# tensorlayer/TLXCV

Measured on AMD Instinct MI355X. Metric: images/sec fwd, higher is better.
Workload: dtype f16; 1 GPU; ResNet-50 fp16 forward, 224x224, batch 256 per GPU (BASELINE configs[1]); global_batch=256, per_gpu_batch=256, weights=seeded random (tlxcv_amd.seeded, seed 1), parallelism=single GPU, launch=hipGraph replay of the forward

## Files before the change

include/tlxmi.h:

```cpp
#ifndef TLXMI_H
#define TLXMI_H

#include <stddef.h>
#include <stdint.h>

#ifdef __cplusplus
extern "C" {
#endif

#define TLXMI_VERSION 101

typedef enum tlxmi_status {
    TLXMI_OK = 0,
    TLXMI_ERR_BAD_ARG = -1,
    TLXMI_ERR_UNSUPPORTED = -2,
    TLXMI_ERR_ALIGNMENT = -3,
    TLXMI_ERR_LAUNCH = -4,
    TLXMI_ERR_NO_DEVICE = -5
} tlxmi_status;

typedef enum tlxmi_dtype { TLXMI_F16 = 0, TLXMI_F32 = 1 } tlxmi_dtype;

typedef enum tlxmi_act {
    TLXMI_ACT_NONE = 0,
// ... 44 lines not shown
    int32_t R, S;
    int32_t stride_h, stride_w, pad_h, pad_w, dil_h, dil_w;
    int32_t Ho, Wo;
    int32_t x_ld, y_ld, res_ld;
    int32_t y_nstride;
    int32_t res_nstride;
    int32_t act;
    float act_param;
    uint32_t flags;
} tlxmi_conv2d_desc;

int tlxmi_conv2d(const tlxmi_conv2d_desc* d, const void* x, const void* w_packed,
                 const float* scale , const float* shift ,
                 const void* res , void* y, void* stream);
int tlxmi_conv2d_maxpool_supported(const tlxmi_conv2d_desc* d);

int tlxmi_yolo_iou_aware(const void* x, void* y, int dtype, int64_t pixels, int A, int C, float factor, void* stream);
int tlxmi_yolo_box(const void* x, int dtype, int N, int A, int C, int H, int W, int channels_last, const int32_t* img_size,
                   const float* anchors, float conf_thresh, int downsample_ratio, int clip_bbox, float scale_x_y,
                   float* boxes, float* scores, int Mtot, int m_offset, void* stream);
size_t tlxmi_multiclass_nms_workspace_bytes(int N, int M);
int tlxmi_multiclass_nms(const float* boxes, const float* scores, int N, int M, int C, float score_threshold, float nms_threshold,
                         int keep_top_k, void* workspace, float* detections, int32_t* counts, void* stream);
int tlxmi_multiclass_nms_index(const float* boxes, const float* scores, int N, int M, int C, float score_threshold,
                               float nms_threshold, int keep_top_k, void* workspace, float* detections, int32_t* counts,
                               int32_t* keep_index, void* stream);

typedef struct tlxmi_preproc_desc {
    int32_t N, H, W, C;
    int32_t out_h, out_w;
    int32_t kh, kw;
    int32_t out_dtype;
    int32_t layout;
    int32_t fold_b, cpad;
    int32_t normalize;
} tlxmi_preproc_desc;
size_t tlxmi_preprocess_u8_workspace_bytes(const tlxmi_preproc_desc* d);
int tlxmi_preprocess_u8(const tlxmi_preproc_desc* d, const void* images, const int32_t* xbounds, const int32_t* xk,
                        const int32_t* ybounds, const int32_t* yk, const float* mean, const float* std_, void* workspace,
                        void* out, void* stream);

int tlxmi_preprocess_linear_u8(const tlxmi_preproc_desc* d, const void* images, const int32_t* xidx, const int32_t* xcoef,
                               const int32_t* yidx, const int32_t* ycoef, const float* mean, const float* std_, void* out,
                               void* stream);

typedef struct tlxmi_seam_desc {
    int32_t dtype;
    int64_t rows;
    int32_t K1, N1, N2;
    int32_t t2_ld, skip_ld, y_ld, t1_ld;
    int32_t act;
} tlxmi_seam_desc;
int tlxmi_bottleneck_seam_supported(int dtype, int K1, int N1, int N2);
int tlxmi_bottleneck_seam_proj(const tlxmi_seam_desc* d, const void* t2, const void* w3_packed, const float* scale3,
                               const float* shift3, const void* x, const void* wd_packed, const float* scale_d,
                               const float* shift_d, void* y, const void* w1_packed, const float* scale1,
                               const float* shift1, void* t1, void* stream);
int tlxmi_bottleneck_seam(const tlxmi_seam_desc* d, const void* t2, const void* w3_packed, const float* scale3,
                          const float* shift3, const void* skip, void* y, const void* w1_packed, const float* scale1,
                          const float* shift1, void* t1, void* stream);
int tlxmi_bottleneck_seam_dec_supported(int dtype, int K1, int N1, int N2, int64_t rows, int H, int W);
int tlxmi_bottleneck_seam_dec(const tlxmi_seam_desc* d, int H, int W, const void* t2, const void* w3_packed, const float* scale3,
                              const float* shift3, const void* skip, void* y, const void* w1_packed, const float* scale1,
                              const float* shift1, void* t1, void* stream);

typedef struct tlxmi_proj_desc {
    int32_t dtype;
    int32_t N, Ho, Wo;
    int32_t K1, K2, Cout;
    int32_t H2, W2, stride;
    int32_t x_ld, x2_ld, y_ld;
    int32_t act;
    float act_param;
    uint32_t flags;
} tlxmi_proj_desc;
int tlxmi_conv1x1_proj_supported(const tlxmi_proj_desc* d, const void* x, const void* x2, const void* w_packed, const void* y);
int tlxmi_conv1x1_proj(const tlxmi_proj_desc* d, const void* x, const void* x2, const void* w_packed, const float* shift, void* y,
                       void* stream);

int tlxmi_group_conv_chunks(int Cin, int Cout, int groups, int dtype);
size_t tlxmi_packed_group_filter_bytes(int Cout, int Cin, int R, int S, int groups, int dtype);
int tlxmi_pack_group_filter(const float* src_oihw, void* dst, int Cout, int Cin, int R, int S, int groups,
                            int dtype, void* stream);
int tlxmi_group_conv2d(const tlxmi_conv2d_desc* d, int groups, const void* x, const void* w_packed,
                       const float* scale, const float* shift, const void* res, void* y, void* stream);
int tlxmi_group_conv2d_small_supported(const tlxmi_conv2d_desc* d, int groups);

int tlxmi_linear_splitk(int dtype, int64_t rows, int K, int Cout, int x_ld, const void* x, const void* w_packed,
                        int splits, void* partials, const float* scale, const float* shift, const void* res,
                        int res_ld, int act, float act_param, uint32_t flags, void* y, int y_ld, void* stream);

int tlxmi_conv2d_splitk_supported(const tlxmi_conv2d_desc* d, int splits);
int tlxmi_conv2d_splitk(const tlxmi_conv2d_desc* d, int splits, const void* x, const void* w_packed, void* partials,
                        const float* scale, const float* shift, const void* res, void* y, void* stream);

typedef struct tlxmi_dwconv2d_desc {
    int32_t dtype;
    int32_t N, H, W, C;
    int32_t R, S, stride_h, stride_w, pad_h, pad_w, dil_h, dil_w;
    int32_t Ho, Wo;
    int32_t x_ld, y_ld;
    int32_t act;
    float act_param;
} tlxmi_dwconv2d_desc;
int tlxmi_dwconv2d(const tlxmi_dwconv2d_desc* d, const void* x, const void* w_rsc, const float* scale,
                   const float* shift, void* y, void* stream);
// ... 222 lines not shown
```

tlxcv_amd/_lib.py:

```python
import ctypes as C
import os

_HERE = os.path.dirname(os.path.abspath(__file__))
LIB_PATH = os.path.join(_HERE, "libtlxmi.so")

F16, F32 = 0, 1
ACT_NONE, ACT_RELU, ACT_RELU6, ACT_LEAKY, ACT_HARDSWISH, ACT_HARDSIGMOID, ACT_GELU, ACT_SIGMOID, ACT_SILU = range(9)
EPI_RES_AFTER_ACT = 1
EPI_MAXPOOL_3S2P1 = 4
PLAN_SHARED_HALF = 0x100
PLAN_SHARED_FULL = 0x200
LAYOUT_NHWC, LAYOUT_NCHW = 0, 1


class ConvDesc(C.Structure):
    _fields_ = [(n, C.c_int32) for n in (
        "dtype", "N", "H", "W", "C", "Cout", "R", "S", "stride_h", "stride_w", "pad_h", "pad_w",
        "dil_h", "dil_w", "Ho", "Wo", "x_ld", "y_ld", "res_ld", "y_nstride", "res_nstride", "act")] + [
        ("act_param", C.c_float), ("flags", C.c_uint32)]


class DwConvDesc(C.Structure):
    _fields_ = [(n, C.c_int32) for n in (
        "dtype", "N", "H", "W", "C", "R", "S", "stride_h", "stride_w", "pad_h", "pad_w", "dil_h",
# ... 114 lines not shown
    "tlxmi_affine_act": [_vp, _vp, _vp, _vp, _vp, _i, _l, _i, _i, _i, _i, _i, _f, _u, _vp],
    "tlxmi_scale_channels": [_vp, _vp, _vp, _i, _i, _i, _i, _i, _i, _i, _vp],
    "tlxmi_layernorm": [_vp, _vp, _vp, _vp, _i, _l, _i, _i, _i, _f, _vp],
    "tlxmi_layernorm_window_partition": [_vp, _vp, _vp, _vp, _i, _i, _i, _i, _i, _i, _i, _f, _vp],
    "tlxmi_window_reverse_layernorm": [_vp, _vp, _vp, _vp, _vp, _vp, _i, _i, _i, _i, _i, _i, _i, _f, _vp],
    "tlxmi_mlp_seam": [_i, _l, _i, _i, _i, _vp, _i, _vp, _vp, _vp, _vp, _vp, _i, _vp, _i, _vp],
    "tlxmi_linear_stats": [_i, _l, _i, _i, _i, _i, _vp, _vp, _vp, _vp, _i, _vp, _vp, _u, _vp],
    "tlxmi_softmax_rows": [_vp, _vp, _i, _l, _i, _l, _l, _vp],
    "tlxmi_linear_ln": [_i, _l, _i, _i, _i, _i, _vp, _vp, _vp, _vp, _vp, _f, _i, _vp, _u, _vp],
    "tlxmi_attention": [C.POINTER(AttnDesc), _vp, _vp, _vp, _vp, _vp],
    "tlxmi_attention_comb": [C.POINTER(AttnDesc), _vp, _vp, _vp, _vp],
    "tlxmi_attention_windows": [C.POINTER(AttnDesc), _vp, _vp, _vp, _i, _i, _i, _i, _vp],
    "tlxmi_mha": [C.POINTER(MhaDesc), _vp, _vp, _vp, _vp, _vp, _vp, _vp],
    "tlxmi_sr_attention": [C.POINTER(MhaDesc), _vp, _vp, _vp, _vp, _vp],
    "tlxmi_cswin_attention": [C.POINTER(CswinAttnDesc), _vp, _vp, _vp, _vp, _vp, _vp, _vp],
    "tlxmi_cswin_attention_plain": [C.POINTER(CswinAttnDesc), _vp, _vp, _vp, _vp, _vp, _vp, _vp],
    "tlxmi_levit_attention": [C.POINTER(LevitAttnDesc), _vp, _vp, _vp, _vp, _vp, _vp],
    "tlxmi_levit_attention_plain": [C.POINTER(LevitAttnDesc), _vp, _vp, _vp, _vp, _vp, _vp],
    "tlxmi_tnt_inner": [C.POINTER(TntInnerDesc), _vp, _vp, _vp, _vp, _vp],
    "tlxmi_tnt_inner_plain": [C.POINTER(TntInnerDesc), _vp, _vp, _vp, _vp, _vp],
    "tlxmi_gsa_block": [C.POINTER(GsaBlockDesc), _vp, _vp, _vp, _vp, _vp, _vp],
    "tlxmi_window_partition": [_vp, _vp, _i, _i, _i, _i, _i, _i, _i, _vp],
    "tlxmi_window_reverse": [_vp, _vp, _vp, _i, _i, _i, _i, _i, _i, _i, _vp],
    "tlxmi_patch_merge_gather": [_vp, _vp, _i, _i, _i, _i, _i, _vp],
    "tlxmi_patch_merge_layernorm": [_vp, _vp, _vp, _vp, _i, _i, _i, _i, _i, _f, _vp],
    "tlxmi_upsample2x_nearest": [_vp, _vp, _i, _i, _i, _i, _i, _i, _i, _i, _vp],
    "tlxmi_copy_channels": [_vp, _vp, _i, _l, _i, _i, _i, _vp],
    "tlxmi_argmax_lastdim": [_vp, _i, _l, _i, _i, _vp, _vp],
    "tlxmi_resize_bilinear": [_vp, _i, _i, _i, _i, _i, _i, _vp, _i, _i, _i, _i, _i, _l, _i, C.c_double, C.c_double, _vp],
    "tlxmi_sepconv2d": [C.POINTER(SepConvDesc), _vp, _vp, _vp, _vp, _vp, _vp, _vp, _vp, _vp],
    "tlxmi_dwconv7_stats": [C.POINTER(DwConv7Desc), _vp, _vp, _vp, _vp, _vp, _vp],
    "tlxmi_preact_conv1x1": [_i, _l, _i, _i, _i, _i, _vp, _vp, _vp, _i, _vp, _vp, _vp, _i, _vp, _vp],
    "tlxmi_lka_dw": [C.POINTER(LkaDwDesc), _vp, _vp, _vp, _vp, _vp, _vp, _vp],
    "tlxmi_lka_gate": [C.POINTER(LkaGateDesc), _vp, _vp, _vp, _vp, _vp, _vp, _vp, _vp, _vp, _vp, _vp, _vp],
    "tlxmi_mul": [_vp, _vp, _vp, _i, _l, _i, _i, _i, _i, _vp],
    "tlxmi_shuffle_unit": [C.POINTER(ShuffleUnitDesc), _vp, _vp, _vp, _vp],
    "tlxmi_shuffle_concat": [_vp, _vp, _vp, _i, _l, _i, _i, _i, _i, _vp],
    "tlxmi_ghost_module": [C.POINTER(GhostModuleDesc), _vp, _vp, _vp, _vp, _vp],
}
_SPECIAL = {
    "tlxmi_version": ([], C.c_int),
    "tlxmi_last_error": ([], C.c_char_p),
    "tlxmi_device_count": ([], C.c_int),
    "tlxmi_packed_filter_bytes": ([_i, _i, _i, _i, _i], C.c_size_t),
    "tlxmi_packed_group_filter_bytes": ([_i, _i, _i, _i, _i, _i], C.c_size_t),
    "tlxmi_group_conv_chunks": ([_i, _i, _i, _i], C.c_int),
    "tlxmi_group_conv2d_small_supported": ([C.POINTER(ConvDesc), _i], C.c_int),
    "tlxmi_conv2d_maxpool_supported": ([C.POINTER(ConvDesc)], C.c_int),
    "tlxmi_conv2d_splitk_supported": ([C.POINTER(ConvDesc), _i], C.c_int),
    "tlxmi_preprocess_u8_workspace_bytes": ([C.POINTER(PreprocDesc)], C.c_size_t),
    "tlxmi_multiclass_nms_workspace_bytes": ([_i, _i], C.c_size_t),
    "tlxmi_bottleneck_seam_supported": ([_i, _i, _i, _i], C.c_int),
    "tlxmi_bottleneck_seam_dec_supported": ([_i, _i, _i, _i, _l, _i, _i], C.c_int),
    "tlxmi_conv1x1_proj_supported": ([C.POINTER(ProjDesc), _vp, _vp, _vp, _vp], C.c_int),
    "tlxmi_linear_ln_supported": ([_i, _l, _i, _i, _i, _i], C.c_int),
    "tlxmi_mlp_seam_supported": ([_i, _i, _i, _i], C.c_int),
    "tlxmi_sepconv2d_supported": ([C.POINTER(SepConvDesc)], C.c_int),
    "tlxmi_dwconv7_stats_supported": ([C.POINTER(DwConv7Desc)], C.c_int),
    "tlxmi_preact_conv1x1_supported": ([_i, _l, _i, _i, _i, _i, _i, _i], C.c_int),
    "tlxmi_sr_attention_supported": ([C.POINTER(MhaDesc)], C.c_int),
    "tlxmi_cswin_attention_supported": ([C.POINTER(CswinAttnDesc)], C.c_int),
    "tlxmi_levit_attention_supported": ([C.POINTER(LevitAttnDesc)], C.c_int),
    "tlxmi_tnt_inner_supported": ([C.POINTER(TntInnerDesc)], C.c_int),
    "tlxmi_tnt_inner_param_count": ([_i, _i], C.c_size_t),
    "tlxmi_gsa_block_supported": ([C.POINTER(GsaBlockDesc)], C.c_int),
    "tlxmi_gsa_block_param_count": ([_i], C.c_size_t),
    "tlxmi_lka_dw_supported": ([C.POINTER(LkaDwDesc)], C.c_int),
    "tlxmi_lka_gate_supported": ([C.POINTER(LkaGateDesc)], C.c_int),
    "tlxmi_shuffle_unit_supported": ([C.POINTER(ShuffleUnitDesc)], C.c_int),
    "tlxmi_shuffle_unit_param_bytes": ([_i], C.c_size_t),
    "tlxmi_ghost_module_supported": ([C.POINTER(GhostModuleDesc)], C.c_int),
    "tlxmi_ghost_module_param_bytes": ([_i, _i], C.c_size_t),
}
ALL_SYMBOLS = sorted(list(PROTOTYPES) + list(_SPECIAL))

TUNE_LIB_PATH = os.environ.get("TLXMI_TUNE_LIB") or os.path.join(_HERE, "libtlxmi_tune.so")

_lib = None
_product = None
_tune = None


def _open(path):
    lib = C.CDLL(path)
    for name, argtypes in PROTOTYPES.items():
        fn = getattr(lib, name)
        fn.argtypes = argtypes
        fn.restype = C.c_int
    for name, (argtypes, restype) in _SPECIAL.items():
        fn = getattr(lib, name)
        fn.argtypes = argtypes
        fn.restype = restype
    return lib


def load():
    global _lib, _product
    if _lib is not None:
        return _lib
    if not os.path.exists(LIB_PATH):
        raise RuntimeError(
            f"tlxcv_amd: {LIB_PATH} is missing — the HIP engine has not been built "
            "(run `python -c 'import __graft_entry__ as g; g.build()'` or `make -C tlxcv_amd/csrc`). "
            "There is no CPU fallback.")
    _product = _open(LIB_PATH)
    _lib = _product
# ... 39 lines not shown
```

tlxcv_amd/csrc/block_seam.h:

```cpp
#pragma once
#include <hip/hip_runtime.h>

namespace tlxmi {

struct SeamArgs {
    const char *x, *w3, *res, *w1;
    char *y, *z;
    const float *scale3, *shift3, *scale1, *shift1;
    int M, N1;
    int x_ld, res_ld, y_ld, z_ld;
    unsigned x_bytes, w3_bytes, res_bytes, y_bytes, w1_bytes, z_bytes;
    int y_nt, z_nt;
    const char* wd;
    const float *scale_d, *shift_d;
    unsigned wd_bytes;
    int debug;
};

struct SeamDecArgs : SeamArgs {
    int HW, W;
};

bool block_seam_shape_ok(int K1, int N1, int N2);
int launch_block_seam(const SeamArgs& a, int K1, int N2, hipStream_t st);
int launch_block_seam_dec(const SeamDecArgs& a, int K1, int N2, hipStream_t st);
int launch_mlp_seam(const SeamArgs& a, int K1, int N2, hipStream_t st);

}
```

tlxcv_amd/csrc/block_seam.hip:

```cpp
#include "kernel_util.h"
#include <stdio.h>
#include "block_seam.h"
#include <type_traits>
#ifdef TLXMI_TUNING
#define TLXMI_DBG_NT(x) (x)
#else
#define TLXMI_DBG_NT(x) (false)
#endif

namespace tlxmi {

static __device__ __forceinline__ int bs_f1(int r) { return ((r >> 1) & 1) | (((r >> 4) & 3) << 1); }
static __device__ __forceinline__ int bs_f2(int r) { return (((r >> 1) & 1) << 2) | ((r >> 5) & 1); }

static __device__ __forceinline__ unsigned bs_pkrelu(unsigned v) {
    unsigned r;
    asm("v_pk_max_f16 %0, %1, 0" : "=v"(r) : "v"(v));
    return r;
}
static __device__ __forceinline__ u32x2 bs_bn_skip_relu4(f32x4 acc, f32x4 sc, f32x4 sh, half4v skip) {
    f32x2 t0 = f32x2{__builtin_fmaf(acc[0], sc[0], (float)skip[0]), __builtin_fmaf(acc[1], sc[1], (float)skip[1])};
    f32x2 t1 = f32x2{__builtin_fmaf(acc[2], sc[2], (float)skip[2]), __builtin_fmaf(acc[3], sc[3], (float)skip[3])};
    t0 += f32x2{sh[0], sh[1]};
    t1 += f32x2{sh[2], sh[3]};
// ... 198 lines not shown
            for (int h = 0; h < 2; ++h) {
                const f32x4 s0 = *reinterpret_cast<const f32x4*>(sc + 8 * h), s1 = *reinterpret_cast<const f32x4*>(sc + 8 * h + 4);
                const f32x4 h0 = *reinterpret_cast<const f32x4*>(sh + 8 * h), h1 = *reinterpret_cast<const f32x4*>(sh + 8 * h + 4);
                f32x4 d0 = s0, d1 = s0, e0 = s0, e1 = s0;
                if constexpr (PROJ) {
                    const float* scd = tabd + 64 * c + 16 * g + 8 * h;
                    d0 = *reinterpret_cast<const f32x4*>(scd); d1 = *reinterpret_cast<const f32x4*>(scd + 4);
                    e0 = *reinterpret_cast<const f32x4*>(scd + a.N1); e1 = *reinterpret_cast<const f32x4*>(scd + a.N1 + 4);
                }
#pragma unroll
                for (int pw = 0; pw < PW; ++pw) {
                    half8v rv;
                    if constexpr (PROJ) {
#pragma unroll
                        for (int e = 0; e < 4; ++e) {
                            rv[e] = (half_t)(accd[2 * h][pw][e] * d0[e] + e0[e]);
                            rv[4 + e] = (half_t)(accd[2 * h + 1][pw][e] * d1[e] + e1[e]);
                        }
                    } else {
                        rv = __builtin_bit_cast(half8v, sk[pw][h]);
                    }
                    if constexpr (MLP) {
                        const u32x2 o0 = bs_bn_gelu4(acc1[2 * h][pw], s0, h0), o1 = bs_bn_gelu4(acc1[2 * h + 1][pw], s1, h1);
                        yf[pw][h] = u32x4{o0[0], o0[1], o1[0], o1[1]};
                        continue;
                    }
                    const u32x2 o0 = bs_bn_skip_relu4(acc1[2 * h][pw], s0, h0, half4v{rv[0], rv[1], rv[2], rv[3]});
                    const u32x2 o1 = bs_bn_skip_relu4(acc1[2 * h + 1][pw], s1, h1, half4v{rv[4], rv[5], rv[6], rv[7]});
                    const u32x4 o = u32x4{o0[0], o0[1], o1[0], o1[1]};
                    yf[pw][h] = o;
                    if (TLXMI_DBG(a, 1)) continue;
                    if constexpr (DEC) {
                        buf_store16(ysrd, yf[pw][h], yoff[pw] + (64 * c + 8 * h) * 2);
                        continue;
                    }
                    if (TLXMI_DBG_NT(a.y_nt)) buf_store16<BUF_NT>(ysrd, yf[pw][h], pok[pw] ? (pix[pw] * a.y_ld + 64 * c + 16 * g + 8 * h) * 2 : BUF_OOB);
                    else buf_store16(ysrd, yf[pw][h], pok[pw] ? (pix[pw] * a.y_ld + 64 * c + 16 * g + 8 * h) * 2 : BUF_OOB);
                }
            }
        }

#pragma unroll
        for (int tt = 0; tt < T2; ++tt) {
            if (TLXMI_DBG(a, 16)) continue;
#pragma unroll
            for (int s = 0; s < 2; ++s) {
                const u32x4 af = *reinterpret_cast<const u32x4*>(wb + (CB + (tt >> 2)) * PANEL + (a2off[tt & 3] ^ (s << 4)));
#pragma unroll
                for (int pw = 0; pw < PW; ++pw) acc2[tt][pw] = Mma<half_t>::run(af, yf[pw][s], acc2[tt][pw]);
            }
        }

        if (more) {
            stage_write((c + 1) & 1, st);
#pragma unroll
            for (int pw = 0; pw < PW; ++pw) { sk[pw][0] = skn[pw][0]; sk[pw][1] = skn[pw][1]; }
        }
        __syncthreads();
    }

#pragma unroll
    for (int q = 0; q < N2 / 64; ++q) {
        const float* sc = tab1 + 64 * q + 16 * g;
        const float* sh = sc + N2;
#pragma unroll
        for (int h = 0; h < 2; ++h) {
            const f32x4 s0 = *reinterpret_cast<const f32x4*>(sc + 8 * h), s1 = *reinterpret_cast<const f32x4*>(sc + 8 * h + 4);
            const f32x4 h0 = *reinterpret_cast<const f32x4*>(sh + 8 * h), h1 = *reinterpret_cast<const f32x4*>(sh + 8 * h + 4);
#pragma unroll
            for (int pw = 0; pw < PW; ++pw) {
                u32x2 o0, o1;
                if constexpr (MLP) {
                    const half8v rv = __builtin_bit_cast(half8v, buf_load16(rsrd, pok[pw] ? (pix[pw] * a.res_ld + 64 * q + 16 * g + 8 * h) * 2 : BUF_OOB));
                    o0 = bs_bn_res4(acc2[4 * q + 2 * h][pw], s0, h0, half4v{rv[0], rv[1], rv[2], rv[3]});
                    o1 = bs_bn_res4(acc2[4 * q + 2 * h + 1][pw], s1, h1, half4v{rv[4], rv[5], rv[6], rv[7]});
                } else {
                    o0 = bs_bn_relu4(acc2[4 * q + 2 * h][pw], s0, h0);
                    o1 = bs_bn_relu4(acc2[4 * q + 2 * h + 1][pw], s1, h1);
                }
                const u32x4 o = u32x4{o0[0], o0[1], o1[0], o1[1]};
                if (TLXMI_DBG(a, 4)) continue;
                if (TLXMI_DBG_NT(a.z_nt)) buf_store16<BUF_NT>(zsrd, o, pok[pw] ? (pix[pw] * a.z_ld + 64 * q + 16 * g + 8 * h) * 2 : BUF_OOB);
                else buf_store16(zsrd, o, pok[pw] ? (pix[pw] * a.z_ld + 64 * q + 16 * g + 8 * h) * 2 : BUF_OOB);
            }
        }
    }
}

template <int K1, int N2, int NW>
__global__ __launch_bounds__(64 * NW, 1) void seam_pair_kernel(const SeamArgs a) {
    static_assert(N2 % 128 == 0 && NW % 2 == 0, "pairs of waves split N2 in halves of whole 64-channel blocks");
    constexpr int NT = 64 * NW;
    constexpr int IPT = 512 / NT;
    constexpr int PW = 2;
    constexpr int KS = K1 / 32;
    constexpr int CB = K1 / 64;
    constexpr int Q2 = N2 / 64;
    constexpr int NP = CB + Q2;
    constexpr int T2H = N2 / 32;
    constexpr int PANEL = 64 * 128;
    extern __shared__ __attribute__((aligned(16))) char smem[];
    char* const wbuf = smem;
    float* const tab3 = reinterpret_cast<float*>(smem + 2 * NP * PANEL);
    float* const tab1 = tab3 + 2 * a.N1;
    char* const ybuf = reinterpret_cast<char*>(tab1 + 2 * N2);

    const int t = threadIdx.x, lane = t & 63;
    const int wid = __builtin_amdgcn_readfirstlane(t >> 6);
    const int hh = wid & 1, pp = wid >> 1;
    const int fr = lane & 15, g = lane >> 4;

// ... 340 lines not shown
            const f32x4 h0 = *reinterpret_cast<const f32x4*>(sh), h1 = *reinterpret_cast<const f32x4*>(sh + 4);
            u32x4 o[PW];
#pragma unroll
            for (int pw = 0; pw < PW; ++pw) {
                const half8v rv = __builtin_bit_cast(half8v, sk[pw]);
                const u32x2 o0 = bs_bn_skip_relu4(acc1[0][pw], s0, h0, half4v{rv[0], rv[1], rv[2], rv[3]});
                const u32x2 o1 = bs_bn_skip_relu4(acc1[1][pw], s1, h1, half4v{rv[4], rv[5], rv[6], rv[7]});
                o[pw] = u32x4{o0[0], o0[1], o1[0], o1[1]};
                if (!TLXMI_DBG(a, 32)) *reinterpret_cast<u32x4*>(ymine + pw * 1024) = o[pw];
                yown[pw] = o[pw];
            }
            skip_load(c + 1, sk, (c + 1 < nch && !TLXMI_DBG(a, 2)) ? 0 : BUF_OOB);
            if (!TLXMI_DBG(a, 1)) {
#pragma unroll
                for (int pw = 0; pw < PW; ++pw) buf_store16(ysrd, o[pw], pok[pw] ? (pix[pw] * a.y_ld + 64 * c + 16 * g + 8 * hh) * 2 : BUF_OOB);
            }
        }
        if constexpr (GRP == 0) wait_vmcnt<4>();
        phase_barrier();
    };
    auto run = [&](auto grp_t) __attribute__((always_inline)) {
        if constexpr (decltype(grp_t)::value == 1) phase_barrier();
        m_phase(0, grp_t, std::true_type{}, std::false_type{});
        n_phase(0, grp_t);
#pragma unroll 1
        for (int c = 1; c < nch; ++c) {
            m_phase(c, grp_t, std::false_type{}, std::false_type{});
            n_phase(c, grp_t);
        }
        m_phase(nch, grp_t, std::false_type{}, std::true_type{});
    };
    if (grp == 0) run(std::integral_constant<int, 0>{});
    else run(std::integral_constant<int, 1>{});

#pragma unroll
    for (int q = 0; q < Q2 / 2; ++q) {
        const float* sc = tab1 + 64 * (hh * (Q2 / 2) + q) + 16 * g;
        const float* sh = sc + N2;
#pragma unroll
        for (int h = 0; h < 2; ++h) {
            const f32x4 s0 = *reinterpret_cast<const f32x4*>(sc + 8 * h), s1 = *reinterpret_cast<const f32x4*>(sc + 8 * h + 4);
            const f32x4 h0 = *reinterpret_cast<const f32x4*>(sh + 8 * h), h1 = *reinterpret_cast<const f32x4*>(sh + 8 * h + 4);
#pragma unroll
            for (int pw = 0; pw < PW; ++pw) {
                const u32x2 o0 = bs_bn_relu4(acc2[4 * q + 2 * h][pw], s0, h0), o1 = bs_bn_relu4(acc2[4 * q + 2 * h + 1][pw], s1, h1);
                const u32x4 o = u32x4{o0[0], o0[1], o1[0], o1[1]};
                buf_store16(zsrd, o, pok[pw] ? (pix[pw] * a.z_ld + 64 * (hh * (Q2 / 2) + q) + 16 * g + 8 * h) * 2 : BUF_OOB);
            }
        }
    }
    if (grp == 0) phase_barrier();
}

constexpr bool SEAM_PAIR_ANTIPHASE = true;

template <int K1, int N2, int NW, bool AP> static int launch_seam_pair_t(const SeamArgs& a, hipStream_t st) {
    static_assert(!AP || NW == 8, "the antiphase form is two groups of four waves");
    constexpr int NP = K1 / 64 + N2 / 64;
    const size_t lds = (size_t)2 * NP * 64 * 128 + (size_t)(2 * a.N1 + 2 * N2) * sizeof(float) + (size_t)NW * 2 * 1024;
    if (lds > 160 * 1024) return fail(TLXMI_ERR_UNSUPPORTED, "block_seam: %zu bytes of LDS", lds);
    const void* fn;
    if constexpr (AP) fn = reinterpret_cast<const void*>(&seam_pair_ap_kernel<K1, N2>);
    else fn = reinterpret_cast<const void*>(&seam_pair_kernel<K1, N2, NW>);
    if (int rc = raise_lds_limit(fn, 160 * 1024, "block_seam")) return rc;
    const long grid = ((long)a.M + NW * 16 - 1) / (NW * 16);
    if (grid >= (1l << 31)) return fail(TLXMI_ERR_UNSUPPORTED, "block_seam: too many rows");
    SeamArgs b = a;
    void* args[] = {&b};
    hipError_t e = hipLaunchKernel(fn, dim3((unsigned)grid), dim3(64 * NW), args, lds, st);
    if (e != hipSuccess) return fail(TLXMI_ERR_LAUNCH, "block_seam: HIP launch failed: %s", hipGetErrorString(e));
    return TLXMI_OK;
}

template <int K1, int N2, int PW, int NW, bool PROJ = false, int WPS = 0, bool MLP = false, bool DEC = false>
static int launch_seam_t(const std::conditional_t<DEC, SeamDecArgs, SeamArgs>& a, hipStream_t st) {
    constexpr int NP = K1 / 64 + N2 / 64 + (PROJ ? K1 / 64 : 0);
    const size_t lds = (size_t)2 * NP * 64 * 128 + (size_t)(2 * a.N1 + 2 * N2 + (PROJ ? 2 * a.N1 : 0)) * sizeof(float);
    if (lds > 160 * 1024) return fail(TLXMI_ERR_UNSUPPORTED, "block_seam: %zu bytes of LDS", lds);
    const void* fn = reinterpret_cast<const void*>(&seam_kernel<K1, N2, PW, NW, PROJ, WPS, MLP, DEC>);
    if (lds > 64 * 1024)
        if (int rc = raise_lds_limit(fn, 160 * 1024, "block_seam")) return rc;
    const long grid = ((long)a.M + NW * 16 * PW - 1) / (NW * 16 * PW);
    if (grid >= (1l << 31)) return fail(TLXMI_ERR_UNSUPPORTED, "block_seam: too many rows");
#ifdef TLXMI_TUNING
    if (tune_int("TLXMI_SEAM_OCC", 0)) {
        int nb = -1;
        hipError_t oe = hipOccupancyMaxActiveBlocksPerMultiprocessor(&nb, fn, 64 * NW, lds);
        fprintf(stderr, "seam<%d,%d,%d,%d,%d>: lds %zu, grid %ld, occupancy %d workgroups / CU (%s)\n", K1, N2, PW, NW, (int)PROJ, lds, grid, nb, hipGetErrorString(oe));
    }
#endif
    auto b = a;
    void* args[] = {&b};
    hipError_t e = hipLaunchKernel(fn, dim3((unsigned)grid), dim3(64 * NW), args, lds, st);
    if (e != hipSuccess) return fail(TLXMI_ERR_LAUNCH, "block_seam: HIP launch failed: %s", hipGetErrorString(e));
    return TLXMI_OK;
}

bool block_seam_shape_ok(int K1, int N1, int N2) {
    if (N1 % 64 || N1 < 64 || N1 > 2048) return false;
    if (!((K1 == 64 && (N2 == 64 || N2 == 128)) || (K1 == 128 && (N2 == 128 || N2 == 256)) || (K1 == 256 && N2 == 256))) return false;
    const size_t lds = (size_t)2 * (K1 / 64 + N2 / 64) * 64 * 128 + (size_t)(2 * N1 + 2 * N2) * sizeof(float) + (K1 == 256 ? (size_t)8 * 2 * 1024 : 0);
    return lds <= 160 * 1024;
}

int launch_mlp_seam(const SeamArgs& a0, int K1, int N2, hipStream_t st) {
    SeamArgs b = a0;
    b.z_nt = b.y_nt = 0;
    b.debug = 0;
    if (K1 == 128 && N2 == 128) return launch_seam_t<128, 128, 2, 8, false, 0, true>(b, st);
    return fail(TLXMI_ERR_UNSUPPORTED, "mlp_seam: no instantiation for %d -> N1 -> %d channels", K1, N2);
}

int launch_block_seam(const SeamArgs& a0, int K1, int N2, hipStream_t st) {
    const int vv = (int)tune_int("TLXMI_SEAM", 0);
    const int v = vv & 1;
    SeamArgs b = a0;
    b.z_nt = (vv & 2) ? 1 : 0;
    b.y_nt = (vv & 4) ? 1 : 0;
    b.debug = (int)tune_int("TLXMI_SEAM_DBG", 0);
    const SeamArgs& a = b;
    if (a.wd) {
        if (K1 == 64 && N2 == 64) return launch_seam_t<64, 64, 2, 4, true>(a, st);
        return fail(TLXMI_ERR_UNSUPPORTED, "block_seam: the projection-shortcut form is compiled for 64 -> N1 -> 64 channels");
    }
    if (vv & 16) {
        if (K1 == 64 && N2 == 64) return launch_seam_t<64, 64, 2, 4, false, 3>(a, st);
        if (K1 == 64 && N2 == 128) return launch_seam_t<64, 128, 2, 4, false, 3>(a, st);
        if (K1 == 128 && N2 == 128) return launch_seam_t<128, 128, 2, 4, false, 2>(a, st);
    }
    if (K1 == 64 && N2 == 64) return v ? launch_seam_t<64, 64, 2, 8>(a, st) : launch_seam_t<64, 64, 2, 4>(a, st);
    if (K1 == 64 && N2 == 128) return v ? launch_seam_t<64, 128, 2, 8>(a, st) : launch_seam_t<64, 128, 2, 4>(a, st);
    if (K1 == 128 && N2 == 128) return v ? launch_seam_t<128, 128, 2, 4>(a, st) : launch_seam_t<128, 128, 2, 8>(a, st);
    if (K1 == 128 && N2 == 256) return v ? launch_seam_t<128, 256, 1, 4>(a, st) : launch_seam_t<128, 256, 1, 8>(a, st);
    if (K1 == 256 && N2 == 256) {
#ifdef TLXMI_TUNING
        if (vv & 64) return launch_seam_pair_t<256, 256, 8, !SEAM_PAIR_ANTIPHASE>(a, st);
#endif
        if (!(vv & 32)) return launch_seam_pair_t<256, 256, 8, SEAM_PAIR_ANTIPHASE>(a, st);
        return v ? launch_seam_t<256, 256, 1, 4>(a, st) : launch_seam_t<256, 256, 1, 8>(a, st);
    }
    return fail(TLXMI_ERR_UNSUPPORTED, "block_seam: no instantiation for %d -> N1 -> %d channels", K1, N2);
}

static bool block_seam_dec_shape_ok(int K1, int N1, int N2) {
    return ((K1 == 64 && N1 == 256 && N2 == 128) || (K1 == 128 && N1 == 512 && N2 == 256)) && block_seam_shape_ok(K1, N1, N2);
}

int launch_block_seam_dec(const SeamDecArgs& a0, int K1, int N2, hipStream_t st) {
    SeamDecArgs b = a0;
    b.z_nt = b.y_nt = 0;
    b.debug = 0;
    if (K1 == 64 && N2 == 128) return launch_seam_t<64, 128, 2, 4, false, 0, false, true>(b, st);
    if (K1 == 128 && N2 == 256) return launch_seam_t<128, 256, 1, 8, false, 0, false, true>(b, st);
    return fail(TLXMI_ERR_UNSUPPORTED, "block_seam_dec: no instantiation for %d -> N1 -> %d channels", K1, N2);
}

}

using namespace tlxmi;

extern "C" int tlxmi_bottleneck_seam_supported(int dtype, int K1, int N1, int N2) {
    return dtype == TLXMI_F16 && block_seam_shape_ok(K1, N1, N2) ? 1 : 0;
}

static int seam_impl(const tlxmi_seam_desc* d, const void* t2, const void* w3_packed, const float* scale3,
                     const float* shift3, const void* skip, void* y, const void* w1_packed, const float* scale1,
                     const float* shift1, void* t1, void* stream, const void* wd_packed, const float* scale_d, const float* shift_d) {
    TLXMI_REQUIRE(d && t2 && w3_packed && skip && y && w1_packed && t1, TLXMI_ERR_BAD_ARG, "bottleneck_seam: null argument");
    TLXMI_REQUIRE(d->dtype == TLXMI_F16, TLXMI_ERR_UNSUPPORTED, "bottleneck_seam: fp16 only (the fp32 parity mode runs the two convolutions)");
    TLXMI_REQUIRE(d->rows > 0 && d->K1 > 0 && d->N1 > 0 && d->N2 > 0, TLXMI_ERR_BAD_ARG, "bottleneck_seam: bad extent");
    if (!block_seam_shape_ok(d->K1, d->N1, d->N2))
        return fail(TLXMI_ERR_UNSUPPORTED, "bottleneck_seam: no kernel for %d -> %d -> %d channels", d->K1, d->N1, d->N2);
    TLXMI_REQUIRE(d->t2_ld >= d->K1 && d->skip_ld >= (wd_packed ? d->K1 : d->N1) && d->y_ld >= d->N1 && d->t1_ld >= d->N2, TLXMI_ERR_BAD_ARG, "bottleneck_seam: row stride below the channel count");
    TLXMI_REQUIRE(!wd_packed || (aligned16(wd_packed) && d->K1 == 64 && d->N2 == 64), TLXMI_ERR_UNSUPPORTED, "bottleneck_seam_proj: 64 -> N1 -> 64 channels only");
    TLXMI_REQUIRE(d->t2_ld % 8 == 0 && d->skip_ld % 8 == 0 && d->y_ld % 8 == 0 && d->t1_ld % 8 == 0 && aligned16(t2) && aligned16(skip) && aligned16(y) &&
                      aligned16(t1) && aligned16(w3_packed) && aligned16(w1_packed),
                  TLXMI_ERR_ALIGNMENT, "bottleneck_seam: rows must be whole 16-byte chunks");
    TLXMI_REQUIRE(d->act == TLXMI_ACT_RELU, TLXMI_ERR_UNSUPPORTED, "bottleneck_seam: ReLU after both convolutions only");
    const long long rows = d->rows;
    const long long big = (1ll << 31);
    TLXMI_REQUIRE(rows * d->t2_ld * 2 < big && rows * d->skip_ld * 2 < big && rows * d->y_ld * 2 < big && rows * d->t1_ld * 2 < big && rows < big,
                  TLXMI_ERR_UNSUPPORTED, "bottleneck_seam: a tensor exceeds the 2 GiB the 32-bit buffer offsets address");
    SeamArgs a;
    a.x = (const char*)t2; a.w3 = (const char*)w3_packed; a.res = (const char*)skip; a.w1 = (const char*)w1_packed;
    a.y = (char*)y; a.z = (char*)t1;
    a.scale3 = scale3; a.shift3 = shift3; a.scale1 = scale1; a.shift1 = shift1;
    a.M = (int)rows; a.N1 = d->N1;
    a.x_ld = d->t2_ld; a.res_ld = d->skip_ld; a.y_ld = d->y_ld; a.z_ld = d->t1_ld;
    a.x_bytes = (unsigned)(rows * d->t2_ld * 2); a.res_bytes = (unsigned)(rows * d->skip_ld * 2);
    a.y_bytes = (unsigned)(rows * d->y_ld * 2); a.z_bytes = (unsigned)(rows * d->t1_ld * 2);
    a.wd = (const char*)wd_packed; a.scale_d = scale_d; a.shift_d = shift_d;
    a.wd_bytes = wd_packed ? (unsigned)(((size_t)(d->N1 + 127) / 128 * 128) * (size_t)d->K1 * 2) : 0u;
    a.w3_bytes = (unsigned)(((size_t)(d->N1 + 127) / 128 * 128) * (size_t)d->K1 * 2);
    a.w1_bytes = (unsigned)(((size_t)(d->N2 + 127) / 128 * 128) * (size_t)d->N1 * 2);
    const int rc = launch_block_seam(a, d->K1, d->N2, as_stream(stream));
    if (rc != TLXMI_OK) return rc;
    return check_launch("bottleneck_seam");
}

extern "C" int tlxmi_bottleneck_seam(const tlxmi_seam_desc* d, const void* t2, const void* w3_packed, const float* scale3,
                                     const float* shift3, const void* skip, void* y, const void* w1_packed, const float* scale1,
                                     const float* shift1, void* t1, void* stream) {
    return seam_impl(d, t2, w3_packed, scale3, shift3, skip, y, w1_packed, scale1, shift1, t1, stream, nullptr, nullptr, nullptr);
}

extern "C" int tlxmi_bottleneck_seam_proj(const tlxmi_seam_desc* d, const void* t2, const void* w3_packed, const float* scale3,
                                          const float* shift3, const void* x, const void* wd_packed, const float* scale_d,
                                          const float* shift_d, void* y, const void* w1_packed, const float* scale1,
                                          const float* shift1, void* t1, void* stream) {
    TLXMI_REQUIRE(wd_packed, TLXMI_ERR_BAD_ARG, "bottleneck_seam_proj: null shortcut filter");
    return seam_impl(d, t2, w3_packed, scale3, shift3, x, y, w1_packed, scale1, shift1, t1, stream, wd_packed, scale_d, shift_d);
}

static long long seam_dec_rows(long long rows, int H, int W) { return rows / ((long long)H * W) * ((H + 1) / 2) * ((W + 1) / 2); }

// ... 72 lines not shown
```

Measured before the change: 80330 images/sec.

## Add persistent seam kernel keeping all bottleneck filters resident in LDS

Adds a persistent kernel for the K1=64 bottleneck seam (conv3 + BN + residual + ReLU fused with the next block's conv1). Each workgroup loads every filter panel and BN table into LDS once, then strides over row tiles, prefetching the next tile's activations during the last channel step. This replaces per-tile re-staging of filters and the double-buffer barriers. In exchange it takes up to 160 KB of LDS per workgroup and caps the grid at a fixed number of workgroups per CU, so occupancy and latency hiding depend on the wave count per workgroup.

After: 80850 images/sec, median of 6. Within noise of the previous version (+0.6%).

```diff
diff --git a/include/tlxmi.h b/include/tlxmi.h
--- a/include/tlxmi.h
+++ b/include/tlxmi.h
@@ -120,6 +120,7 @@
     int32_t act;
 } tlxmi_seam_desc;
 int tlxmi_bottleneck_seam_supported(int dtype, int K1, int N1, int N2);
+int tlxmi_bottleneck_seam_resident(int dtype, int K1, int N1, int N2, int proj);
 int tlxmi_bottleneck_seam_proj(const tlxmi_seam_desc* d, const void* t2, const void* w3_packed, const float* scale3,
                                const float* shift3, const void* x, const void* wd_packed, const float* scale_d,
                                const float* shift_d, void* y, const void* w1_packed, const float* scale1,
diff --git a/tlxcv_amd/_lib.py b/tlxcv_amd/_lib.py
--- a/tlxcv_amd/_lib.py
+++ b/tlxcv_amd/_lib.py
@@ -190,6 +190,7 @@
     "tlxmi_multiclass_nms_workspace_bytes": ([_i, _i], C.c_size_t),
     "tlxmi_bottleneck_seam_supported": ([_i, _i, _i, _i], C.c_int),
     "tlxmi_bottleneck_seam_dec_supported": ([_i, _i, _i, _i, _l, _i, _i], C.c_int),
+    "tlxmi_bottleneck_seam_resident": ([_i, _i, _i, _i, _i], C.c_int),
     "tlxmi_conv1x1_proj_supported": ([C.POINTER(ProjDesc), _vp, _vp, _vp, _vp], C.c_int),
     "tlxmi_linear_ln_supported": ([_i, _l, _i, _i, _i, _i], C.c_int),
     "tlxmi_mlp_seam_supported": ([_i, _i, _i, _i], C.c_int),
diff --git a/tlxcv_amd/csrc/block_seam.h b/tlxcv_amd/csrc/block_seam.h
--- a/tlxcv_amd/csrc/block_seam.h
+++ b/tlxcv_amd/csrc/block_seam.h
@@ -22,6 +22,7 @@
 };
 
 bool block_seam_shape_ok(int K1, int N1, int N2);
+bool block_seam_resident_ok(int K1, int N1, int N2, bool proj);
 int launch_block_seam(const SeamArgs& a, int K1, int N2, hipStream_t st);
 int launch_block_seam_dec(const SeamDecArgs& a, int K1, int N2, hipStream_t st);
 int launch_mlp_seam(const SeamArgs& a, int K1, int N2, hipStream_t st);
diff --git a/tlxcv_amd/csrc/block_seam.hip b/tlxcv_amd/csrc/block_seam.hip
--- a/tlxcv_amd/csrc/block_seam.hip
+++ b/tlxcv_amd/csrc/block_seam.hip
@@ -274,11 +274,11 @@
         }
 
         if (more) {
-            stage_write((c + 1) & 1, st);
+            if (!TLXMI_DBG(a, 128)) stage_write((c + 1) & 1, st);
 #pragma unroll
             for (int pw = 0; pw < PW; ++pw) { sk[pw][0] = skn[pw][0]; sk[pw][1] = skn[pw][1]; }
         }
-        __syncthreads();
+        if (!TLXMI_DBG(a, 64)) __syncthreads();
     }
 
 #pragma unroll
@@ -725,6 +725,306 @@
     if (grp == 0) phase_barrier();
 }
 
+template <bool DEC> using SeamArgsOf = std::conditional_t<DEC, SeamDecArgs, SeamArgs>;
+
+template <int K1, int N2, int PW, int NW, bool PROJ = false, bool DEC = false, int NCH = 0>
+__global__ __launch_bounds__(64 * NW, 1) void seam_resident_kernel(const SeamArgsOf<DEC> a) {
+    static_assert(!(DEC && PROJ), "the decimated store belongs to the plain seam");
+    constexpr int NT = 64 * NW;
+    constexpr int IPT = (512 + NT - 1) / NT;
+    constexpr int KS = K1 / 32;
+    constexpr int CB = K1 / 64;
+    constexpr int Q2 = N2 / 64;
+    constexpr int CD = PROJ ? CB : 0;
+    constexpr int NP = CB + Q2 + CD;
+    constexpr int T2 = N2 / 16;
+    constexpr int PANEL = 64 * 128;
+    constexpr int TILE = 16 * PW;
+    constexpr int FB = 4;
+    extern __shared__ __attribute__((aligned(16))) char smem[];
+    const int nch = NCH ? NCH : a.N1 >> 6;
+    char* const wbuf = smem;
+    float* const tab3 = reinterpret_cast<float*>(smem + nch * NP * PANEL);
+    float* const tab1 = tab3 + 2 * a.N1;
+    float* const tabd = tab1 + 2 * N2;
+
+    const int t = threadIdx.x, lane = t & 63;
+    const int wid = __builtin_amdgcn_readfirstlane(t >> 6);
+    const int fr = lane & 15, g = lane >> 4;
+
+    const __amdgpu_buffer_rsrc_t xsrd = buf_srd(a.x, a.x_bytes), w3srd = buf_srd(a.w3, a.w3_bytes), w1srd = buf_srd(a.w1, a.w1_bytes);
+    const __amdgpu_buffer_rsrc_t rsrd = buf_srd(a.res, a.res_bytes), ysrd = buf_srd(a.y, a.y_bytes), zsrd = buf_srd(a.z, a.z_bytes);
+    const __amdgpu_buffer_rsrc_t wdsrd = buf_srd(PROJ ? a.wd : a.w3, PROJ ? a.wd_bytes : 0u);
+
+    const int ntiles = (a.M + TILE - 1) / TILE;
+    const int tstride = (int)gridDim.x * NW;
+    int tile = (int)blockIdx.x * NW + wid;
+    int xb[PW], rb[PW], yb[PW], zb[PW];
+    auto tile_offsets = [&](int tl, int (&xo)[PW], int (&ro)[PW]) __attribute__((always_inline)) {
+#pragma unroll
+        for (int pw = 0; pw < PW; ++pw) {
+            const int p = tl * TILE + 16 * pw + fr;
+            const bool ok = p < a.M;
+            xo[pw] = ok ? (p * a.x_ld + 8 * g) * 2 : BUF_OOB;
+            ro[pw] = ok ? (p * a.res_ld + (PROJ ? 8 : 16) * g) * 2 : BUF_OOB;
+        }
+    };
+    auto tile_out_offsets = [&](int tl) __attribute__((always_inline)) {
+#pragma unroll
+        for (int pw = 0; pw < PW; ++pw) {
+            const int p = tl * TILE + 16 * pw + fr;
+            const bool ok = p < a.M;
+            if constexpr (!DEC) yb[pw] = ok ? (p * a.y_ld + 16 * g) * 2 : BUF_OOB;
+            zb[pw] = ok ? (p * a.z_ld + 16 * g) * 2 : BUF_OOB;
+        }
+    };
+    auto frag_load = [&](const int (&xo)[PW], const int (&ro)[PW], u32x4 (&xv)[KS][PW], u32x4 (&xpv)[PROJ ? KS : 1][PW]) __attribute__((always_inline)) {
+#pragma unroll
+        for (int pw = 0; pw < PW; ++pw)
+#pragma unroll
+            for (int ks = 0; ks < KS; ++ks) xv[ks][pw] = buf_load16(xsrd, xo[pw] + 64 * ks);
+        if constexpr (PROJ) {
+#pragma unroll
+            for (int pw = 0; pw < PW; ++pw)
+#pragma unroll
+                for (int ks = 0; ks < KS; ++ks) xpv[ks][pw] = buf_load16(rsrd, ro[pw] + 64 * ks);
+        }
+    };
+    auto skip_load = [&](const int (&ro)[PW], int c, u32x4 (&s)[PW][2]) __attribute__((always_inline)) {
+        if constexpr (PROJ) return;
+#pragma unroll
+        for (int pw = 0; pw < PW; ++pw)
+#pragma unroll
+            for (int h = 0; h < 2; ++h) s[pw][h] = buf_load16(rsrd, ro[pw] + (64 * c + 8 * h) * 2);
+    };
+
+    u32x4 xf[KS][PW], xpf[PROJ ? KS : 1][PW], sk[PW][2];
+    tile_offsets(tile, xb, rb);
+    frag_load(xb, rb, xf, xpf);
+    skip_load(rb, 0, sk);
+
+    for (int c0 = 0; c0 < nch; c0 += FB) {
+        u32x4 st[FB][NP][IPT];
+#pragma unroll
+        for (int i = 0; i < FB; ++i) {
+            const int c = c0 + i;
+#pragma unroll
+            for (int k = 0; k < IPT; ++k) {
+                const int idx = k * NT + t, srow = idx >> 3, sslot = idx & 7;
+                const int dead = (c < nch && idx < 512) ? 0 : BUF_OOB;
+                const int sl1 = sslot ^ bs_f1(srow), sl2 = sslot ^ bs_f2(srow);
+#pragma unroll
+                for (int cb = 0; cb < CB; ++cb) st[i][cb][k] = buf_load16(w3srd, (((64 * c + srow) * K1 + 64 * cb + 8 * sl1) * 2) | dead);
+#pragma unroll
+                for (int q = 0; q < Q2; ++q) st[i][CB + q][k] = buf_load16(w1srd, (((64 * q + srow) * a.N1 + 64 * c + 8 * sl2) * 2) | dead);
+#pragma unroll
+                for (int cb = 0; cb < CD; ++cb) st[i][CB + Q2 + cb][k] = buf_load16(wdsrd, (((64 * c + srow) * K1 + 64 * cb + 8 * sl1) * 2) | dead);
+            }
+        }
+#pragma unroll
+        for (int i = 0; i < FB; ++i) {
+            if (c0 + i >= nch) break;
+#pragma unroll
+            for (int j = 0; j < NP; ++j)
+#pragma unroll
+                for (int k = 0; k < IPT; ++k)
+                    if (k * NT + t < 512) *reinterpret_cast<u32x4*>(wbuf + ((c0 + i) * NP + j) * PANEL + (k * NT + t) * 16) = st[i][j][k];
+        }
+    }
+    for (int i = t; i < a.N1; i += NT) {
+        tab3[i] = a.scale3 ? a.scale3[i] : 1.f;
+        tab3[a.N1 + i] = a.shift3 ? a.shift3[i] : 0.f;
+    }
+    for (int i = t; i < N2; i += NT) {
+        tab1[i] = a.scale1 ? a.scale1[i] : 1.f;
+        tab1[N2 + i] = a.shift1 ? a.shift1[i] : 0.f;
+    }
+    if constexpr (PROJ) {
+        for (int i = t; i < a.N1; i += NT) {
+            tabd[i] = a.scale_d ? a.scale_d[i] : 1.f;
+            tabd[a.N1 + i] = a.shift_d ? a.shift_d[i] : 0.f;
+        }
+    }
+    __builtin_amdgcn_s_waitcnt(0x0F70);
+    __syncthreads();
+
+    const int arow = 16 * (fr >> 2) + (fr & 3);
+    int a1off[4], a2off[4];
+#pragma unroll
+    for (int ci = 0; ci < 4; ++ci) {
+        const int r = arow + 4 * ci;
+        a1off[ci] = r * 128 + ((g ^ bs_f1(r)) << 4);
+        a2off[ci] = r * 128 + (((2 * g) ^ bs_f2(r)) << 4);
+    }
+
+    int dn_[DEC ? PW : 1], dh_[DEC ? PW : 1], dw_[DEC ? PW : 1];
+    int sn = 0, sh_ = 0, sw = 0, Hh = 1, Wc = 1, HcWc = 1;
+    if constexpr (DEC) {
+        Hh = a.HW / a.W;
+        Wc = (a.W + 1) >> 1;
+        HcWc = ((Hh + 1) >> 1) * Wc;
+        const int S = tstride * TILE, sr = S % a.HW;
+        sn = S / a.HW; sh_ = sr / a.W; sw = sr - sh_ * a.W;
+#pragma unroll
+        for (int pw = 0; pw < PW; ++pw) {
+            const int p = tile * TILE + 16 * pw + fr, n = p / a.HW, r = p - n * a.HW, h = r / a.W;
+            dn_[pw] = n; dh_[pw] = h; dw_[pw] = r - h * a.W;
+        }
+    }
+
+#pragma unroll 1
+    for (; tile < ntiles; tile += tstride) {
+        tile_out_offsets(tile);
+        if constexpr (DEC) {
+#pragma unroll
+            for (int pw = 0; pw < PW; ++pw) {
+                const bool keep = tile * TILE + 16 * pw + fr < a.M && !((dh_[pw] | dw_[pw]) & 1);
+                yb[pw] = keep ? ((dn_[pw] * HcWc + (dh_[pw] >> 1) * Wc + (dw_[pw] >> 1)) * a.y_ld + 16 * g) * 2 : BUF_OOB;
+            }
+        }
+        int xbn[PW], rbn[PW];
+        tile_offsets(tile + tstride, xbn, rbn);
+
+        f32x4 acc2[T2][PW];
+#pragma unroll
+        for (int tt = 0; tt < T2; ++tt)
+#pragma unroll
+            for (int pw = 0; pw < PW; ++pw) acc2[tt][pw] = f32x4{0.f, 0.f, 0.f, 0.f};
+
+        auto step = [&](int c, auto last_t) __attribute__((always_inline)) {
+            constexpr bool LAST = decltype(last_t)::value;
+            const char* const wb = wbuf + c * NP * PANEL;
+            u32x4 skn[PW][2];
+            if (!TLXMI_DBG(a, 2)) {
+                if constexpr (LAST) skip_load(rbn, 0, skn);
+                else skip_load(rb, c + 1, skn);
+            }
+            __builtin_amdgcn_sched_barrier(0);
+
+            f32x4 acc1[4][PW];
+#pragma unroll
+            for (int ci = 0; ci < 4; ++ci) {
+#pragma unroll
+                for (int pw = 0; pw < PW; ++pw) acc1[ci][pw] = f32x4{0.f, 0.f, 0.f, 0.f};
+                if (TLXMI_DBG(a, 16)) continue;
+#pragma unroll
+                for (int ks = 0; ks < KS; ++ks) {
+                    const u32x4 af = *reinterpret_cast<const u32x4*>(wb + (ks >> 1) * PANEL + (a1off[ci] ^ ((ks & 1) << 6)));
+#pragma unroll
+                    for (int pw = 0; pw < PW; ++pw) acc1[ci][pw] = Mma<half_t>::run(af, xf[ks][pw], acc1[ci][pw]);
+                }
+            }
+            f32x4 accd[PROJ ? 4 : 1][PW];
+            if constexpr (PROJ) {
+#pragma unroll
+                for (int ci = 0; ci < 4; ++ci) {
+#pragma unroll
+                    for (int pw = 0; pw < PW; ++pw) accd[ci][pw] = f32x4{0.f, 0.f, 0.f, 0.f};
+#pragma unroll
+                    for (int ks = 0; ks < KS; ++ks) {
+                        const u32x4 af = *reinterpret_cast<const u32x4*>(wb + (CB + Q2 + (ks >> 1)) * PANEL + (a1off[ci] ^ ((ks & 1) << 6)));
+#pragma unroll
+                        for (int pw = 0; pw < PW; ++pw) accd[ci][pw] = Mma<half_t>::run(af, xpf[ks][pw], accd[ci][pw]);
+                    }
+                }
+            }
+            if constexpr (LAST) {
+                __builtin_amdgcn_sched_barrier(0);
+                frag_load(xbn, rbn, xf, xpf);
+                __builtin_amdgcn_sched_barrier(0);
+            }
+
+            u32x4 yf[PW][2];
+            {
+                const float* sc = tab3 + 64 * c + 16 * g;
+                const float* sh = sc + a.N1;
+#pragma unroll
+                for (int h = 0; h < 2; ++h) {
+                    const f32x4 s0 = *reinterpret_cast<const f32x4*>(sc + 8 * h), s1 = *reinterpret_cast<const f32x4*>(sc + 8 * h + 4);
+                    const f32x4 h0 = *reinterpret_cast<const f32x4*>(sh + 8 * h), h1 = *reinterpret_cast<const f32x4*>(sh + 8 * h + 4);
+                    f32x4 d0 = s0, d1 = s0, e0 = s0, e1 = s0;
+                    if constexpr (PROJ) {
+                        const float* scd = tabd + 64 * c + 16 * g + 8 * h;
+                        d0 = *reinterpret_cast<const f32x4*>(scd); d1 = *reinterpret_cast<const f32x4*>(scd + 4);
+                        e0 = *reinterpret_cast<const f32x4*>(scd + a.N1); e1 = *reinterpret_cast<const f32x4*>(scd + a.N1 + 4);
+                    }
+#pragma unroll
+                    for (int pw = 0; pw < PW; ++pw) {
+                        half8v rv;
+                        if constexpr (PROJ) {
+#pragma unroll
+                            for (int e = 0; e < 4; ++e) {
+                                rv[e] = (half_t)(accd[2 * h][pw][e] * d0[e] + e0[e]);
+                                rv[4 + e] = (half_t)(accd[2 * h + 1][pw][e] * d1[e] + e1[e]);
+                            }
+                        } else {
+                            rv = __builtin_bit_cast(half8v, sk[pw][h]);
+                        }
+                        const u32x2 o0 = bs_bn_skip_relu4(acc1[2 * h][pw], s0, h0, half4v{rv[0], rv[1], rv[2], rv[3]});
+                        const u32x2 o1 = bs_bn_skip_relu4(acc1[2 * h + 1][pw], s1, h1, half4v{rv[4], rv[5], rv[6], rv[7]});
+                        yf[pw][h] = u32x4{o0[0], o0[1], o1[0], o1[1]};
+                        if (TLXMI_DBG(a, 1)) continue;
+                        buf_store16(ysrd, yf[pw][h], yb[pw] + (64 * c + 8 * h) * 2);
+                    }
+                }
+            }
+
+#pragma unroll
+            for (int tt = 0; tt < T2; ++tt) {
+                if (TLXMI_DBG(a, 16)) continue;
+#pragma unroll
+                for (int s = 0; s < 2; ++s) {
+                    const u32x4 af = *reinterpret_cast<const u32x4*>(wb + (CB + (tt >> 2)) * PANEL + (a2off[tt & 3] ^ (s << 4)));
+#pragma unroll
+                    for (int pw = 0; pw < PW; ++pw) acc2[tt][pw] = Mma<half_t>::run(af, yf[pw][s], acc2[tt][pw]);
+                }
+            }
+            if constexpr (!PROJ) {
+#pragma unroll
+                for (int pw = 0; pw < PW; ++pw) { sk[pw][0] = skn[pw][0]; sk[pw][1] = skn[pw][1]; }
+            }
+        };
+        if constexpr (NCH > 0) {
+#pragma unroll
+            for (int c = 0; c < NCH - 1; ++c) step(c, std::false_type{});
+        } else {
+#pragma unroll 1
+            for (int c = 0; c + 1 < nch; ++c) step(c, std::false_type{});
+        }
+        step(nch - 1, std::true_type{});
+
+#pragma unroll
+        for (int q = 0; q < Q2; ++q) {
+            const float* sc = tab1 + 64 * q + 16 * g;
+            const float* sh = sc + N2;
+#pragma unroll
+            for (int h = 0; h < 2; ++h) {
+                const f32x4 s0 = *reinterpret_cast<const f32x4*>(sc + 8 * h), s1 = *reinterpret_cast<const f32x4*>(sc + 8 * h + 4);
+                const f32x4 h0 = *reinterpret_cast<const f32x4*>(sh + 8 * h), h1 = *reinterpret_cast<const f32x4*>(sh + 8 * h + 4);
+#pragma unroll
+                for (int pw = 0; pw < PW; ++pw) {
+                    const u32x2 o0 = bs_bn_relu4(acc2[4 * q + 2 * h][pw], s0, h0), o1 = bs_bn_relu4(acc2[4 * q + 2 * h + 1][pw], s1, h1);
+                    if (TLXMI_DBG(a, 4)) continue;
+                    buf_store16(zsrd, u32x4{o0[0], o0[1], o1[0], o1[1]}, zb[pw] + (64 * q + 8 * h) * 2);
+                }
+            }
+        }
+
+#pragma unroll
+        for (int pw = 0; pw < PW; ++pw) {
+            rb[pw] = rbn[pw];
+            if constexpr (DEC) {
+                int w = dw_[pw] + sw, h = dh_[pw] + sh_, n = dn_[pw] + sn;
+                const int cw = w >= a.W ? 1 : 0;
+                w -= cw ? a.W : 0; h += cw;
+                const int ch = h >= Hh ? 1 : 0;
+                h -= ch ? Hh : 0; n += ch;
+                dn_[pw] = n; dh_[pw] = h; dw_[pw] = w;
+            }
+        }
+    }
+}
+
 constexpr bool SEAM_PAIR_ANTIPHASE = true;
 
 template <int K1, int N2, int NW, bool AP> static int launch_seam_pair_t(const SeamArgs& a, hipStream_t st) {
@@ -769,6 +1069,53 @@
     return TLXMI_OK;
 }
 
+static size_t seam_resident_lds(int K1, int N1, int N2, bool proj) {
+    const size_t np = (size_t)(K1 / 64 + N2 / 64 + (proj ? K1 / 64 : 0));
+    return np * (size_t)(N1 / 64) * 64 * 128 + (size_t)(2 * N1 + 2 * N2 + (proj ? 2 * N1 : 0)) * sizeof(float);
+}
+
+bool block_seam_resident_ok(int K1, int N1, int N2, bool proj) {
+    if (K1 != 64 || N1 % 64 || N1 < 64) return false;
+    if (!(N2 == 64 || (N2 == 128 && !proj))) return false;
+    return seam_resident_lds(K1, N1, N2, proj) <= 160 * 1024;
+}
+
+constexpr int SEAM_RESIDENT_WG_PER_CU = 4;
+
+template <int K1, int N2, int PW, int NW, bool PROJ = false, bool DEC = false>
+static int launch_seam_resident_t(const SeamArgsOf<DEC>& a, hipStream_t st) {
+    const size_t lds = seam_resident_lds(K1, a.N1, N2, PROJ);
+    if (lds > 160 * 1024) return fail(TLXMI_ERR_UNSUPPORTED, "block_seam: %zu bytes of LDS for resident filters", lds);
+    const void* fn = a.N1 == 256 ? reinterpret_cast<const void*>(&seam_resident_kernel<K1, N2, PW, NW, PROJ, DEC, 4>)
+                                 : reinterpret_cast<const void*>(&seam_resident_kernel<K1, N2, PW, NW, PROJ, DEC, 0>);
+    if (lds > 64 * 1024)
+        if (int rc = raise_lds_limit(fn, 160 * 1024, "block_seam")) return rc;
+    const long ntiles = ((long)a.M + 16 * PW - 1) / (16 * PW);
+    long grid = (ntiles + NW - 1) / NW;
+    long cap = (long)SEAM_RESIDENT_WG_PER_CU * device_cus();
+    if (const long forced = tune_int("TLXMI_SEAM_GRID", 0); forced > 0) cap = forced;
+    if (grid > cap) grid = cap;
+    auto b = a;
+    void* args[] = {&b};
+    hipError_t e = hipLaunchKernel(fn, dim3((unsigned)grid), dim3(64 * NW), args, lds, st);
+    if (e != hipSuccess) return fail(TLXMI_ERR_LAUNCH, "block_seam: HIP launch failed: %s", hipGetErrorString(e));
+    return TLXMI_OK;
+}
+
+static bool seam_resident_rows_ok(int M, int tune_bits) {
+    if ((tune_bits & 256) || tune_int("TLXMI_SEAM_GRID", 0) > 0) return true;
+    return ((long)M + 31) / 32 > (long)SEAM_RESIDENT_WG_PER_CU * device_cus() * 8;
+}
+
+template <int N2, bool PROJ, bool DEC> static int launch_seam_resident(const SeamArgsOf<DEC>& a, hipStream_t st) {
+#ifdef TLXMI_TUNING
+    const long shape = tune_int("TLXMI_SEAM_RES", 0);
+    if (shape == 1) return launch_seam_resident_t<64, N2, 1, 16, PROJ, DEC>(a, st);
+    if (shape == 2) return launch_seam_resident_t<64, N2, 2, 12, PROJ, DEC>(a, st);
+#endif
+    return launch_seam_resident_t<64, N2, 2, 8, PROJ, DEC>(a, st);
+}
+
 bool block_seam_shape_ok(int K1, int N1, int N2) {
     if (N1 % 64 || N1 < 64 || N1 > 2048) return false;
     if (!((K1 == 64 && (N2 == 64 || N2 == 128)) || (K1 == 128 && (N2 == 128 || N2 == 256)) || (K1 == 256 && N2 == 256))) return false;
@@ -792,6 +1139,11 @@
     b.y_nt = (vv & 4) ? 1 : 0;
     b.debug = (int)tune_int("TLXMI_SEAM_DBG", 0);
     const SeamArgs& a = b;
+    if (!(vv & 128) && block_seam_resident_ok(K1, a.N1, N2, a.wd != nullptr) && seam_resident_rows_ok(a.M, vv)) {
+        if (a.wd) return launch_seam_resident<64, true, false>(a, st);
+        if (N2 == 64) return launch_seam_resident<64, false, false>(a, st);
+        return launch_seam_resident<128, false, false>(a, st);
+    }
     if (a.wd) {
         if (K1 == 64 && N2 == 64) return launch_seam_t<64, 64, 2, 4, true>(a, st);
         return fail(TLXMI_ERR_UNSUPPORTED, "block_seam: the projection-shortcut form is compiled for 64 -> N1 -> 64 channels");
@@ -822,7 +1174,10 @@
 int launch_block_seam_dec(const SeamDecArgs& a0, int K1, int N2, hipStream_t st) {
     SeamDecArgs b = a0;
     b.z_nt = b.y_nt = 0;
-    b.debug = 0;
+    b.debug = (int)tune_int("TLXMI_SEAM_DBG", 0);
+    const int vv = (int)tune_int("TLXMI_SEAM", 0);
+    if (!(vv & 128) && N2 == 128 && block_seam_resident_ok(K1, b.N1, N2, false) && seam_resident_rows_ok(b.M, vv))
+        return launch_seam_resident<128, false, true>(b, st);
     if (K1 == 64 && N2 == 128) return launch_seam_t<64, 128, 2, 4, false, 0, false, true>(b, st);
     if (K1 == 128 && N2 == 256) return launch_seam_t<128, 256, 1, 8, false, 0, false, true>(b, st);
     return fail(TLXMI_ERR_UNSUPPORTED, "block_seam_dec: no instantiation for %d -> N1 -> %d channels", K1, N2);
@@ -834,6 +1189,11 @@
 
 extern "C" int tlxmi_bottleneck_seam_supported(int dtype, int K1, int N1, int N2) {
     return dtype == TLXMI_F16 && block_seam_shape_ok(K1, N1, N2) ? 1 : 0;
+}
+
+extern "C" int tlxmi_bottleneck_seam_resident(int dtype, int K1, int N1, int N2, int proj) {
+    if (dtype != TLXMI_F16 || !block_seam_shape_ok(K1, N1, N2) || (proj && !(K1 == 64 && N2 == 64))) return 0;
+    return block_seam_resident_ok(K1, N1, N2, proj != 0) ? 1 : 0;
 }
 
 static int seam_impl(const tlxmi_seam_desc* d, const void* t2, const void* w3_packed, const float* scale3,
```
